# ZhonghuaYi/FocusFlow_official

Measured on AMD Instinct MI355X. Metric: frame-pairs/sec FF-RAFT 384x512 iters=12, higher is better.
Workload: dtype f32 via fp16x3 split operands on the f16 MFMA pipe (f32 accumulate, fp32-level accuracy); 1 GPU; FF-RAFT forward (test_mode), 8 pairs/GPU 384x512, iters=12, fp32 correlation pyramid, random-init weights, ORB-like masks (BASELINE configs[1]); pairs_per_gpu=8, corr_pyramid=fp32, conv_precision=f16x3, hipgraph=False, skip_unused_upsample=False, parallelism=dp1 (independent shards, no collective)

## Files before the change

### focusflow_official_amd/csrc/conv_small.hip

```cpp
#include "ff_common.h"

namespace {

constexpr int RUN = 8;

struct SArgs {
    FFConvParams p;
    int Cin, runs_x;
};

__device__ __forceinline__ float dot4(const f32x4 a, const f32x4 b, float acc) {
    acc = fmaf(a[0], b[0], acc); acc = fmaf(a[1], b[1], acc); acc = fmaf(a[2], b[2], acc); return fmaf(a[3], b[3], acc);
}

template <int COUT>
__global__ __launch_bounds__(256) void conv_small_kernel(const SArgs a) {
    const FFConvParams& p = a.p;
    const int lane = threadIdx.x & 63;
    const long long task = (long long)blockIdx.x * 4 + (threadIdx.x >> 6);
    const long long ntask = (long long)p.B * p.H * a.runs_x;
    if (task >= ntask) return;
    const int run = (int)(task % a.runs_x);
    const int y = (int)((task / a.runs_x) % p.H);
    const int b = (int)(task / ((long long)a.runs_x * p.H));
    const int x0 = run * RUN;
    const int H = p.H, W = p.W, K = 9 * a.Cin;

    float mine[COUT];
#pragma unroll
    for (int c = 0; c < COUT; ++c) mine[c] = 0.f;

    for (int cbase = 0; cbase < a.Cin; cbase += 256) {
        const int cpos = cbase + lane * 4;
        const bool cok = cpos < a.Cin;
        const float* xp = p.x[0];
        int ld = p.x_ld[0], cs = 0;
        if (cok) {
            const int c0 = p.x_c[0], c01 = p.x_c[0] + p.x_c[1];
            cs = cpos;
            if (cs < c0) { xp = p.x[0]; ld = p.x_ld[0]; }
            else if (cs < c01) { xp = p.x[1]; ld = p.x_ld[1]; cs -= c0; }
            else { xp = p.x[2]; ld = p.x_ld[2]; cs -= c01; }
        }
        f32x4 w[COUT][9];
#pragma unroll
        for (int c = 0; c < COUT; ++c)
#pragma unroll
            for (int t = 0; t < 9; ++t)
                w[c][t] = cok ? *reinterpret_cast<const f32x4*>(p.w + (long long)c * K + t * a.Cin + cpos) : (f32x4){0.f, 0.f, 0.f, 0.f};
        auto load = [&](int yy, int xx) {
            const bool ok = cok && (unsigned)yy < (unsigned)H && (unsigned)xx < (unsigned)W;
            const int yc = min(max(yy, 0), H - 1), xc = min(max(xx, 0), W - 1);
            const f32x4 v = *reinterpret_cast<const f32x4*>(xp + ((long long)(b * H + yc) * W + xc) * ld + cs);
            return ok ? v : (f32x4){0.f, 0.f, 0.f, 0.f};
        };
        f32x4 col[3][3];
#pragma unroll
        for (int dy = 0; dy < 3; ++dy) { col[0][dy] = load(y - 1 + dy, x0 - 1); col[1][dy] = load(y - 1 + dy, x0); }
#pragma unroll
        for (int i = 0; i < RUN; ++i) {
#pragma unroll
            for (int dy = 0; dy < 3; ++dy) col[(i + 2) % 3][dy] = load(y - 1 + dy, x0 + i + 1);
#pragma unroll
            for (int c = 0; c < COUT; ++c) {
                float s = 0.f;
#pragma unroll
                for (int dy = 0; dy < 3; ++dy)
#pragma unroll
                    for (int dx = 0; dx < 3; ++dx) s = dot4(col[(i + dx) % 3][dy], w[c][dy * 3 + dx], s);
#pragma unroll
                for (int o = 32; o > 0; o >>= 1) s += __shfl_xor(s, o);
                if (lane == i) mine[c] += s;
            }
        }
    }
    const int x = x0 + lane;
    if (lane < RUN && x < W) {
        const long long m = ((long long)b * H + y) * W + x;
#pragma unroll
        for (int c = 0; c < COUT; ++c) {
            float v = mine[c] + (p.bias ? p.bias[c] : 0.f);
            v *= p.out_scale;
            if (p.ch_scale) v = v * p.ch_scale[c] + p.ch_shift[c];
            v = ff::apply_act(v, p.act);
            if (p.res) v = ff::apply_act(v + p.res[m * p.res_ld + c], p.act_res);
            p.y[m * p.y_ld + c] = v;
            mine[c] = v;
        }
        if constexpr (COUT == 2) {
            if (p.ep_mode == FF_EP_COORDS) {
                float* c1 = const_cast<float*>(p.ep_a) + m * 2;
                const float cx = __fadd_rn(c1[0], mine[0]), cy = __fadd_rn(c1[1], mine[1]);
                c1[0] = cx;
                c1[1] = cy;
                *reinterpret_cast<f32x4*>(const_cast<float*>(p.ep_b) + m * 4) = (f32x4){__fsub_rn(cx, (float)x), __fsub_rn(cy, (float)y), 0.f, 0.f};
            }
        }
    }
}

}

namespace ff {
int conv2d_fwd_small(const FFConvParams& p, int cin, hipStream_t s) {
    const int dlh = p.dil_h ? p.dil_h : 1, dlw = p.dil_w ? p.dil_w : 1;
    if (p.w_format != FF_W_F32 || p.Cout > 2 || p.KH != 3 || p.KW != 3 || p.stride != 1 || p.pad_h != 1 || p.pad_w != 1 ||
        dlh != 1 || dlw != 1 || p.groups != 1)
        return 1;
    SArgs a;
    a.p = p;
    a.Cin = cin;
    a.runs_x = (p.W + RUN - 1) / RUN;
    const long long tasks = (long long)p.B * p.H * a.runs_x;
    const unsigned blocks = (unsigned)((tasks + 3) / 4);
    if (p.Cout == 1) conv_small_kernel<1><<<blocks, 256, 0, s>>>(a);
    else conv_small_kernel<2><<<blocks, 256, 0, s>>>(a);
    return check_launch("ff_conv2d_fwd(small)");
}
}

namespace {

struct DArgs {
    const float* x; int x_ld;
    const float* w;
    const float* bias;
    float* y; int y_ld;
    int B, H, W, Cin, runs_x;
};

template <int COUT>
__global__ __launch_bounds__(256) void deconv4x4s2_small_kernel(const DArgs a) {
    const int lane = threadIdx.x & 63;
    const int Ho = 2 * a.H, Wo = 2 * a.W;
    const long long task = (long long)blockIdx.x * 4 + (threadIdx.x >> 6);
    if (task >= (long long)a.B * Ho * a.runs_x) return;
    const int run = (int)(task % a.runs_x);
    const int oy = (int)((task / a.runs_x) % Ho);
    const int b = (int)(task / ((long long)a.runs_x * Ho));
    const int ox0 = run * RUN, n0 = ox0 >> 1;
    const int a0 = oy & 1;
    const int iy0 = (oy - 2 + a0) >> 1;
    const int K = 16 * a.Cin;

    float mine[COUT];
#pragma unroll
    for (int c = 0; c < COUT; ++c) mine[c] = 0.f;
    for (int cbase = 0; cbase < a.Cin; cbase += 256) {
        const int cpos = cbase + lane * 4;
        const bool cok = cpos < a.Cin;
        f32x4 w[COUT][2][4];
#pragma unroll
        for (int c = 0; c < COUT; ++c)
#pragma unroll
            for (int r = 0; r < 2; ++r)
#pragma unroll
                for (int bb = 0; bb < 4; ++bb)
                    w[c][r][bb] = cok ? *reinterpret_cast<const f32x4*>(a.w + (long long)c * K + ((a0 + 2 * r) * 4 + bb) * a.Cin + cpos)
                                      : (f32x4){0.f, 0.f, 0.f, 0.f};
        auto load = [&](int iy, int ix) {
            const bool ok = cok && (unsigned)iy < (unsigned)a.H && (unsigned)ix < (unsigned)a.W;
            const int yc = min(max(iy, 0), a.H - 1), xc = min(max(ix, 0), a.W - 1);
            const f32x4 v = *reinterpret_cast<const f32x4*>(a.x + ((long long)(b * a.H + yc) * a.W + xc) * a.x_ld + (cok ? cpos : 0));
            return ok ? v : (f32x4){0.f, 0.f, 0.f, 0.f};
        };
        f32x4 col[6][2];
#pragma unroll
        for (int j = 0; j < 6; ++j)
#pragma unroll
            for (int r = 0; r < 2; ++r) col[j][r] = load(iy0 + r, n0 - 1 + j);
#pragma unroll
        for (int i = 0; i < RUN; ++i) {
            const int b0 = i & 1, j0 = ((i - 2 + b0) >> 1) + 1;
#pragma unroll
            for (int c = 0; c < COUT; ++c) {
                float s = 0.f;
#pragma unroll
                for (int r = 0; r < 2; ++r)
#pragma unroll
                    for (int t = 0; t < 2; ++t) s = dot4(col[j0 + t][r], w[c][r][b0 + 2 * t], s);
#pragma unroll
                for (int o = 32; o > 0; o >>= 1) s += __shfl_xor(s, o);
                if (lane == i) mine[c] += s;
            }
        }
    }
    const int ox = ox0 + lane;
    if (lane < RUN && ox < Wo) {
        const long long m = ((long long)b * Ho + oy) * Wo + ox;
#pragma unroll
        for (int c = 0; c < COUT; ++c) a.y[m * a.y_ld + c] = mine[c] + (a.bias ? a.bias[c] : 0.f);
    }
}

}

extern "C" int ff_deconv4x4s2_small(const float* x, int x_ld, int B, int H, int W, int Cin, const float* w, const float* bias,
                                    int Cout, float* y, int y_ld, void* stream) {
    FF_REQUIRE(x && w && y && B > 0 && H > 0 && W > 0 && Cin > 0 && Cin % 4 == 0 && (Cout == 1 || Cout == 2),
               "ff_deconv4x4s2_small: Cin must be a multiple of 4, Cout 1 or 2");
    FF_REQUIRE(x_ld >= Cin && x_ld % 4 == 0 && y_ld >= Cout && ff::aligned16(x) && ff::aligned16(w), "ff_deconv4x4s2_small: ld/alignment");
    DArgs a;
    a.x = x; a.x_ld = x_ld; a.w = w; a.bias = bias; a.y = y; a.y_ld = y_ld;
    a.B = B; a.H = H; a.W = W; a.Cin = Cin;
    a.runs_x = (2 * W + RUN - 1) / RUN;
    const long long tasks = (long long)B * 2 * H * a.runs_x;
    const unsigned blocks = (unsigned)((tasks + 3) / 4);
    hipStream_t s = static_cast<hipStream_t>(stream);
    if (Cout == 1) deconv4x4s2_small_kernel<1><<<blocks, 256, 0, s>>>(a);
    else deconv4x4s2_small_kernel<2><<<blocks, 256, 0, s>>>(a);
    return ff::check_launch("ff_deconv4x4s2_small");
}
```

Baseline: 628.3 frame-pairs/s.

## Add MFMA halo-tile kernel for 3x3 convs with one or two output channels

Adds a tiled kernel for small-Cout 3x3 convolutions with Cin>=128. Each block covers a 6x8 output tile plus halo and computes per-pixel, per-tap partial products with f32 16x16x4 MFMA, treating the 9 or 18 tap-channel columns as the N dimension. Partials are then summed across waves and shifted taps through shared memory. This replaces the per-pixel FMA dot products and 64-lane shuffle reductions of the old kernel with matrix-core work and halo reuse. In exchange it recomputes halo pixels, does redundant padded MFMA columns for Cout=1, and adds an LDS reduction plus a __syncthreads.

```diff
diff --git a/focusflow_official_amd/csrc/conv_small.hip b/focusflow_official_amd/csrc/conv_small.hip
--- a/focusflow_official_amd/csrc/conv_small.hip
+++ b/focusflow_official_amd/csrc/conv_small.hip
@@ -11,6 +11,51 @@
 
 __device__ __forceinline__ float dot4(const f32x4 a, const f32x4 b, float acc) {
     acc = fmaf(a[0], b[0], acc); acc = fmaf(a[1], b[1], acc); acc = fmaf(a[2], b[2], acc); return fmaf(a[3], b[3], acc);
+}
+
+template <int COUT>
+struct EpOps {
+    float bias[COUT], res[COUT], c1[2];
+};
+
+template <int COUT>
+__device__ __forceinline__ EpOps<COUT> load_ep(const FFConvParams& p, int b, int y, int x) {
+    const long long m = ((long long)b * p.H + y) * p.W + x;
+    EpOps<COUT> e;
+#pragma unroll
+    for (int c = 0; c < COUT; ++c) {
+        e.bias[c] = p.bias ? p.bias[c] : 0.f;
+        e.res[c] = p.res ? p.res[m * p.res_ld + c] : 0.f;
+    }
+    e.c1[0] = e.c1[1] = 0.f;
+    if constexpr (COUT == 2) {
+        if (p.ep_mode == FF_EP_COORDS) { e.c1[0] = p.ep_a[m * 2]; e.c1[1] = p.ep_a[m * 2 + 1]; }
+    }
+    return e;
+}
+
+template <int COUT>
+__device__ __forceinline__ void finish_pixel(const FFConvParams& p, int b, int y, int x, float (&mine)[COUT], const EpOps<COUT>& e) {
+    const long long m = ((long long)b * p.H + y) * p.W + x;
+#pragma unroll
+    for (int c = 0; c < COUT; ++c) {
+        float v = mine[c] + e.bias[c];
+        v *= p.out_scale;
+        if (p.ch_scale) v = v * p.ch_scale[c] + p.ch_shift[c];
+        v = ff::apply_act(v, p.act);
+        if (p.res) v = ff::apply_act(v + e.res[c], p.act_res);
+        p.y[m * p.y_ld + c] = v;
+        mine[c] = v;
+    }
+    if constexpr (COUT == 2) {
+        if (p.ep_mode == FF_EP_COORDS) {
+            float* c1 = const_cast<float*>(p.ep_a) + m * 2;
+            const float cx = __fadd_rn(e.c1[0], mine[0]), cy = __fadd_rn(e.c1[1], mine[1]);
+            c1[0] = cx;
+            c1[1] = cy;
+            *reinterpret_cast<f32x4*>(const_cast<float*>(p.ep_b) + m * 4) = (f32x4){__fsub_rn(cx, (float)x), __fsub_rn(cy, (float)y), 0.f, 0.f};
+        }
+    }
 }
 
 template <int COUT>
@@ -75,27 +120,129 @@
         }
     }
     const int x = x0 + lane;
-    if (lane < RUN && x < W) {
-        const long long m = ((long long)b * H + y) * W + x;
+    if (lane < RUN && x < W) finish_pixel<COUT>(p, b, y, x, mine, load_ep<COUT>(p, b, y, x));
+}
+
+constexpr int TH = 6, TW = 8, HALO_W = TW + 2, NPIX = (TH + 2) * HALO_W, NGRP = NPIX / 16, SLAB_LD = 20;
+static_assert(NPIX % 16 == 0, "the halo tile is whole groups of 16 pixels");
+
+struct TArgs {
+    FFConvParams p;
+    int Cin, tiles_x, tiles_y;
+};
+
+template <int COUT>
+__global__ __launch_bounds__(256) void conv_small_tile_kernel(const TArgs a) {
+    __shared__ float slab[4][NPIX][SLAB_LD];
+    constexpr int NCOL = COUT == 2 ? 16 : 9, NEXT = COUT == 2 ? 2 : 0;
+    const FFConvParams& p = a.p;
+    const int lane = threadIdx.x & 63, wv = __builtin_amdgcn_readfirstlane(threadIdx.x >> 6);
+    const int pi = lane & 15, kq = lane >> 4;
+    const int nblk = gridDim.x, q8 = nblk / 8, r8 = nblk % 8, cls = blockIdx.x % 8;
+    const int tile = (cls < r8 ? cls * (q8 + 1) : r8 * (q8 + 1) + (cls - r8) * q8) + blockIdx.x / 8;
+    const int tx = tile % a.tiles_x, ty = (tile / a.tiles_x) % a.tiles_y, b = tile / (a.tiles_x * a.tiles_y);
+    const int y0 = ty * TH, x0 = tx * TW, H = p.H, W = p.W, Cin = a.Cin;
+
+    int pix[NGRP];
+#pragma unroll
+    for (int g = 0; g < NGRP; ++g) {
+        const int q = g * 16 + pi, iy = y0 - 1 + q / HALO_W, ix = x0 - 1 + q % HALO_W;
+        pix[g] = (b * H + min(max(iy, 0), H - 1)) * W + min(max(ix, 0), W - 1);
+    }
+    f32x4 acc[NGRP];
+    float ext[NGRP][NEXT > 0 ? NEXT : 1];
+#pragma unroll
+    for (int g = 0; g < NGRP; ++g) {
+        acc[g] = (f32x4){0.f, 0.f, 0.f, 0.f};
+#pragma unroll
+        for (int e = 0; e < NEXT; ++e) ext[g][e] = 0.f;
+    }
+
+    const int c0 = p.x_c[0], c01 = p.x_c[0] + p.x_c[1];
+    for (int cbase = wv * 64; cbase < Cin; cbase += 256) {
+        const float* xp[4];
+        long long ld[4];
+        f32x4 bw[4], wx[4][NEXT > 0 ? NEXT : 1];
+        float keep[4];
+#pragma unroll
+        for (int j = 0; j < 4; ++j) {
+            const int cpos = cbase + j * 16 + kq * 4;
+            const bool cok = cpos < Cin;
+            const int seg = cpos < c0 ? 0 : (cpos < c01 ? 1 : 2);
+            const int cs = cpos - (seg == 0 ? 0 : (seg == 1 ? c0 : c01));
+            xp[j] = cok ? (seg == 0 ? p.x[0] : (seg == 1 ? p.x[1] : p.x[2])) + cs : p.w;
+            ld[j] = cok ? (seg == 0 ? p.x_ld[0] : (seg == 1 ? p.x_ld[1] : p.x_ld[2])) : 0;
+            keep[j] = cok ? 1.f : 0.f;
+            const float* wc = p.w + (cok ? cpos : 0);
+            bw[j] = *reinterpret_cast<const f32x4*>(wc + (long long)min(pi, NCOL - 1) * Cin);
+#pragma unroll
+            for (int e = 0; e < NEXT; ++e) wx[j][e] = *reinterpret_cast<const f32x4*>(wc + (long long)(16 + e) * Cin);
+        }
+        f32x4 xa[NGRP][4];
+#pragma unroll
+        for (int g = 0; g < NGRP; ++g)
+#pragma unroll
+            for (int j = 0; j < 4; ++j) xa[g][j] = *reinterpret_cast<const f32x4*>(xp[j] + pix[g] * ld[j]);
+        __builtin_amdgcn_sched_barrier(0);
+#pragma unroll
+        for (int j = 0; j < 4; ++j) {
+            bw[j] *= keep[j];
+#pragma unroll
+            for (int e = 0; e < NEXT; ++e) wx[j][e] *= keep[j];
+        }
+#pragma unroll
+        for (int g0 = 0; g0 < NGRP; g0 += 2) {
+#pragma unroll
+            for (int j = 0; j < 4; ++j) {
+#pragma unroll
+                for (int t = 0; t < 4; ++t)
+#pragma unroll
+                    for (int g = g0; g < g0 + 2 && g < NGRP; ++g)
+                        acc[g] = __builtin_amdgcn_mfma_f32_16x16x4f32(xa[g][j][t], bw[j][t], acc[g], 0, 0, 0);
+#pragma unroll
+                for (int g = g0; g < g0 + 2 && g < NGRP; ++g)
+#pragma unroll
+                    for (int e = 0; e < NEXT; ++e) ext[g][e] = dot4(xa[g][j], wx[j][e], ext[g][e]);
+            }
+            __builtin_amdgcn_sched_barrier(0);
+        }
+    }
+    const int oy = threadIdx.x / TW, ox = threadIdx.x % TW, y = y0 + oy, x = x0 + ox;
+    const bool has_px = oy < TH && y < H && x < W;
+    EpOps<COUT> eo = {};
+    if (has_px) eo = load_ep<COUT>(p, b, y, x);
+#pragma unroll
+    for (int g = 0; g < NGRP; ++g) {
+        if (pi < NCOL) {
+#pragma unroll
+            for (int r = 0; r < 4; ++r) slab[wv][g * 16 + kq * 4 + r][pi] = acc[g][r];
+        }
+#pragma unroll
+        for (int e = 0; e < NEXT; ++e) {
+            float s = ext[g][e];
+            s += __shfl_xor(s, 16);
+            s += __shfl_xor(s, 32);
+            if (kq == 0) slab[wv][g * 16 + pi][16 + e] = s;
+        }
+    }
+    __syncthreads();
+    if (has_px) {
+        float mine[COUT];
 #pragma unroll
         for (int c = 0; c < COUT; ++c) {
-            float v = mine[c] + (p.bias ? p.bias[c] : 0.f);
-            v *= p.out_scale;
-            if (p.ch_scale) v = v * p.ch_scale[c] + p.ch_shift[c];
-            v = ff::apply_act(v, p.act);
-            if (p.res) v = ff::apply_act(v + p.res[m * p.res_ld + c], p.act_res);
-            p.y[m * p.y_ld + c] = v;
-            mine[c] = v;
-        }
-        if constexpr (COUT == 2) {
-            if (p.ep_mode == FF_EP_COORDS) {
-                float* c1 = const_cast<float*>(p.ep_a) + m * 2;
-                const float cx = __fadd_rn(c1[0], mine[0]), cy = __fadd_rn(c1[1], mine[1]);
-                c1[0] = cx;
-                c1[1] = cy;
-                *reinterpret_cast<f32x4*>(const_cast<float*>(p.ep_b) + m * 4) = (f32x4){__fsub_rn(cx, (float)x), __fsub_rn(cy, (float)y), 0.f, 0.f};
+            float s = 0.f;
+#pragma unroll
+            for (int t = 0; t < 9; ++t) {
+                const bool in = (unsigned)(y - 1 + t / 3) < (unsigned)H && (unsigned)(x - 1 + t % 3) < (unsigned)W;
+#pragma unroll
+                for (int w4 = 0; w4 < 4; ++w4) {
+                    const float v = slab[w4][(oy + t / 3) * HALO_W + ox + t % 3][c * 9 + t];
+                    s += in ? v : 0.f;
+                }
             }
-        }
+            mine[c] = s;
+        }
+        finish_pixel<COUT>(p, b, y, x, mine, eo);
     }
 }
 
@@ -107,6 +254,18 @@
     if (p.w_format != FF_W_F32 || p.Cout > 2 || p.KH != 3 || p.KW != 3 || p.stride != 1 || p.pad_h != 1 || p.pad_w != 1 ||
         dlh != 1 || dlw != 1 || p.groups != 1)
         return 1;
+    static const bool tile_enabled = !(getenv("FF_SMALL_TILE") && atoi(getenv("FF_SMALL_TILE")) == 0);
+    if (tile_enabled && cin >= 128) {
+        TArgs t;
+        t.p = p;
+        t.Cin = cin;
+        t.tiles_x = (p.W + TW - 1) / TW;
+        t.tiles_y = (p.H + TH - 1) / TH;
+        const unsigned blocks = (unsigned)((long long)p.B * t.tiles_y * t.tiles_x);
+        if (p.Cout == 1) conv_small_tile_kernel<1><<<blocks, 256, 0, s>>>(t);
+        else conv_small_tile_kernel<2><<<blocks, 256, 0, s>>>(t);
+        return check_launch("ff_conv2d_fwd(small, tile)");
+    }
     SArgs a;
     a.p = p;
     a.Cin = cin;
```

Measured after the change: 635.0 frame-pairs/s (median of 6 runs). +1.1%, better.
